# rdpoor/pygmu2

Hardware: AMD Instinct MI355X
Metric: Msamples/s rendered (benchmark_pes.py metric: output frames / wall second) (higher is better)
Workload: dtype f64; 1 GPU; C2: BiquadPE(SinePE(440), lowpass 1 kHz, q 0.707), 44.1 kHz mono, render(start, 1_000_000) per step; frames_counted=11287000000, parallelism=single chain, c2_process_warmup_streams=10

## Files before the change

include/pygmu_hip.h:

```cpp
#ifndef PYGMU_HIP_H
#define PYGMU_HIP_H

#include <stddef.h>
#include <stdint.h>

#define PGX_HOST

#ifdef __cplusplus
extern "C" {
#endif

typedef enum {
    PGX_OK = 0,
    PGX_ERR_INVALID = -1,
    PGX_ERR_RUNTIME = -2,
    PGX_ERR_NOT_INIT = -3,
    PGX_ERR_NOMEM = -4
} pgx_status;

int pgx_abi_version(void);
const char *pgx_last_error(void);
int pgx_device_count(PGX_HOST int *count);
int pgx_init(int device);
int pgx_shutdown(void);
// ... 60 lines not shown
    int32_t pad;
} pgx_sine_stateful_params;
int pgx_sine_stateful(float *out, int64_t n, int channels, double sample_rate,
                      const pgx_sine_stateful_params *params,
                      const float *freq, const float *amp, const float *phase_mod,
                      double *state );

size_t pgx_sine_stateful_bank_workspace_bytes(int64_t n, int batch);
int pgx_sine_stateful_bank(float *out, int64_t out_stride, int batch, int64_t n, int channels, double sample_rate,
                           const pgx_sine_stateful_params *params ,
                           const float *freq, int64_t freq_stride, const float *amp, int64_t amp_stride,
                           const float *phase_mod, int64_t phase_stride,
                           double *state , void *workspace );

int pgx_gain_const(float *out, const float *in, int64_t n_elems, float gain);
int pgx_gain_vec(float *out, const float *in, const float *gain, int64_t n, int channels,
                 int gain_channels );
int pgx_mix_n(float *out, PGX_HOST const float *const *ins_host, int k, int64_t n_elems);
int pgx_mix_batch(float *out, const float *in, int64_t in_stride, int batch, int64_t n_elems);
int pgx_gain_mix_batch(float *out, const float *in, int64_t in_stride, const float *gain,
                       int64_t gain_stride, int batch, int64_t n, int channels, int gain_channels);

size_t pgx_biquad_workspace_bytes(int batch, int64_t n, int channels, int64_t settle_frames);
size_t pgx_biquad_table_doubles(void);
int pgx_biquad_tables(double *tables, const double *coef , int batch);
int pgx_biquad_const(float *out, int64_t out_stride, const float *in, int64_t in_stride,
                     int batch, int64_t n, int channels,
                     const double *coef , const double *tables, int64_t settle_frames,
                     double *state , void *workspace);

int pgx_biquad_sine_supported(int64_t n, int64_t settle_frames);
int pgx_biquad_sine(float *out, int64_t start, int64_t n, double sample_rate, double w, double amp, double phase0,
                    const double *coef , const double *tables, int64_t settle_frames,
                    double *state ,
                    double *state_backup );
int pgx_biquad_sine_set_runs(int min_chunks);
int pgx_biquad_sine_runs_plan(int64_t n, int64_t settle_frames, PGX_HOST int out[5]);
int pgx_biquad_sine_set_pacing(int mode);
int pgx_biquad_sine_pacing_info(int64_t out[3]);

int pgx_biquad_tone_supported(int64_t n, int64_t settle_frames, double w, double sample_rate, double b0, double b1,
                              double b2, double a1, double a2);
double pgx_biquad_tone_gain(double w, double sample_rate, double b0, double b1, double b2, double a1, double a2);
double pgx_biquad_tone_l1(int64_t settle_frames, double b0, double b1, double b2, double a1, double a2);
int pgx_biquad_tone(float *out, int64_t start, int64_t n, double sample_rate, double w, double amp, double phase0,
                    double b0, double b1, double b2, double a1, double a2, const double *tables,
                    int64_t settle_frames, double *state , double *state_backup );
int64_t pgx_biquad_tone_window_frames(void);
void *pgx_biquad_tone_plan(double sample_rate, double w, double amp, double phase0, double b0, double b1, double b2,
                           double a1, double a2, const double *tables, int64_t settle_frames);
int pgx_biquad_tone_plan_free(void *plan);
int pgx_biquad_tone_window(const void *plan, float *out, int64_t start, int64_t n, double *state ,
                           double *state_backup );

typedef struct {
    double freq;
    double q;
    double gain_db;
    int32_t mode;
    int32_t pad;
} pgx_biquad_var_params;
size_t pgx_scan2_workspace_bytes(int64_t n, int channels);
int pgx_biquad_varying(float *out, const float *in, int64_t n, int channels, double sample_rate,
                       const pgx_biquad_var_params *params, const float *freq, const float *q,
                       double gain_a, double gain_sqrt_a, double *state ,
                       void *workspace);
int pgx_biquad_varying_bank(float *out, int64_t out_stride, const float *in, int64_t in_stride, int batch, int64_t n,
                            int channels, double sample_rate, const pgx_biquad_var_params *params, const double *gains,
                            const float *freq, int64_t freq_stride, const float *q, int64_t q_stride,
                            double *state, void *workspace);

int pgx_svf(float *out, const float *in, int64_t n, int channels, double sample_rate,
            const pgx_biquad_var_params *params, const float *freq, const float *q, double gain_a,
            const double *coef ,
            double *state , void *workspace );
int pgx_svf_bank(float *out, int64_t out_stride, const float *in, int64_t in_stride, int batch, int64_t n, int channels,
                 double sample_rate, const pgx_biquad_var_params *params, const double *gains,
                 const float *freq, int64_t freq_stride, const float *q, int64_t q_stride, const double *coef,
                 double *state, void *workspace);

size_t pgx_envelope_scratch_bytes(int64_t n, int channels);
int pgx_envelope(float *out, const float *in, int64_t n, int channels, double attack_coeff,
                 double release_coeff, int one_pole, int rms_window, int64_t rms_period, double *state,
                 double *scratch);

typedef struct {
    int32_t code;
    int32_t pad;
    double p0;
    double p1;
} pgx_transform_op;
int pgx_transform(float *out, const float *in, int64_t n_elems, const pgx_transform_op *ops, int nops);
int pgx_transform_bank(float *out, const float *in, int64_t per_voice, int batch, const pgx_transform_op *ops,
                       int nops);

typedef struct {
    int32_t code;
    int32_t tuning;
    double p0;
    double p1;
} pgx_tuning_op;
typedef struct {
    double reference_pitch;
    double reference_freq;
    double divisions;
    int64_t table_offset;
// ... 375 lines not shown
```

pygmu2_amd/biquad_pe.py:

```python

from __future__ import annotations

from enum import Enum

import ctypes
import math
import os

import numpy as np

from . import device as _dev
from . import diagnostics as _diag
from ._kernels import DeviceBuffer, check, lib, new_output, ptr
from .config import handle_error
from .extent import Extent
from .processing_element import ProcessingElement
from .sine_pe import SinePE
from .snippet import Snippet

FUSE_SINE_SOURCE = True
SINE_FAST_RANGE = 2.0e9
TONE_WINDOWS = os.environ.get("PYGMU_BIQUAD_TONE", "1") != "0"


def tone_window_frames() -> int:
    return int(_dev.load_library().pgx_biquad_tone_window_frames())


class _TonePlan:
    __slots__ = ("handle",)

    def __init__(self, handle):
        self.handle = handle

    def __del__(self):
        handle, self.handle = self.handle, None
        if handle:
            try:
                _dev.load_library().pgx_biquad_tone_plan_free(handle)
            except Exception:
                pass


class BiquadMode(Enum):
    LOWPASS = "lowpass"
    HIGHPASS = "highpass"
    BANDPASS = "bandpass"
    NOTCH = "notch"
    ALLPASS = "allpass"
    PEAKING = "peaking"
    LOWSHELF = "lowshelf"
    HIGHSHELF = "highshelf"


_MODE_INDEX = {m: i for i, m in enumerate(BiquadMode)}


def rbj_coefficients(mode: BiquadMode, freq: float, q: float, gain_db: float, sample_rate: float):
    f = np.atleast_1d(freq).astype(np.float64)
    qq = np.atleast_1d(q).astype(np.float64)
    nyquist = sample_rate / 2.0
    f = np.clip(f, 1.0, nyquist * 0.99)
    qq = np.clip(qq, 0.01, 100.0)
    omega = 2.0 * np.pi * f / sample_rate
    sn, cs = np.sin(omega), np.cos(omega)
    alpha = sn / (2.0 * qq)
    A = 10.0 ** (gain_db / 40.0)
    if mode == BiquadMode.LOWPASS:
        b0 = (1.0 - cs) / 2.0; b1 = 1.0 - cs; b2 = (1.0 - cs) / 2.0
        a0 = 1.0 + alpha; a1 = -2.0 * cs; a2 = 1.0 - alpha
    elif mode == BiquadMode.HIGHPASS:
        b0 = (1.0 + cs) / 2.0; b1 = -(1.0 + cs); b2 = (1.0 + cs) / 2.0
        a0 = 1.0 + alpha; a1 = -2.0 * cs; a2 = 1.0 - alpha
    elif mode == BiquadMode.BANDPASS:
        b0 = alpha; b1 = 0.0; b2 = -alpha
        a0 = 1.0 + alpha; a1 = -2.0 * cs; a2 = 1.0 - alpha
    elif mode == BiquadMode.NOTCH:
        b0 = 1.0; b1 = -2.0 * cs; b2 = 1.0
        a0 = 1.0 + alpha; a1 = -2.0 * cs; a2 = 1.0 - alpha
# ... 135 lines not shown
            self._state.zero_()

    _on_start = _reset_state
    _on_stop = _reset_state

    def _ensure_state(self, channels: int) -> None:
        if self._state is None or self._state_channels != channels:
            per = 4 if (self._freq_is_pe or self._q_is_pe) else 2
            self._state = DeviceBuffer((channels, per), np.float64, zero=True)
            self._state_channels = channels

    def _prepare_constant(self, L, sr: float) -> None:
        if self._coef is None:
            coef = rbj_coefficients(self._mode, self._frequency, self._q, self._gain_db, sr)
            self._coef = DeviceBuffer.from_host(np.asarray(coef, dtype=np.float64))
            self._coef_host = tuple(float(c) for c in coef)
            self._settle = settle_frames(coef[3], coef[4])
            if self._settle:
                self._tables = DeviceBuffer((L.pgx_biquad_table_doubles(),), np.float64)
                check(L.pgx_biquad_tables(self._tables.ptr, self._coef.ptr, 1), "pgx_biquad_tables")

    def _sine_chain(self):
        if self._sine_chain_memo is None:
            src, chain = self._source, False
            if (not self._freq_is_pe and not self._q_is_pe and type(src) is SinePE and not src._has_pe_inputs()
                    and src._channels == 1):
                L = lib()
                sr = float(self.sample_rate)
                self._prepare_constant(L, sr)
                w = 2.0 * np.pi * float(src._frequency)
                if self._settle and _passes_more_signal_than_rounding(self._coef_host, w / sr, self._settle):
                    chain = (w, float(src._amplitude), float(src._phase))
            self._sine_chain_memo = chain
        return self._sine_chain_memo or None

    def _render_sine_source(self, start: int, duration: int):
        if not FUSE_SINE_SOURCE or _diag.is_enabled():
            return None
        chain = self._sine_chain()
        if chain is None:
            return None
        w, amp, phase = chain
        L = lib()
        sr = float(self.sample_rate)
        ok = self._sine_supported.get(duration)
        if ok is None:
            ok = self._sine_supported[duration] = bool(L.pgx_biquad_sine_supported(duration, self._settle))
        if not ok or abs(phase) + abs(w) * ((abs(start) + duration) / sr) >= SINE_FAST_RANGE:
            return None
        self._ensure_state(1)
        out = new_output(duration, 1)
        backup, self._backup_target = self._backup_target, None
        if self._takes_tone_window(L, start, duration, w, phase, sr):
            plan = self._tone_plan
            if plan is None:
                plan = self._tone_plan = _TonePlan(L.pgx_biquad_tone_plan(sr, w, amp, phase, *self._coef_host,
                                                                          self._tables.ptr, self._settle))
            check(L.pgx_biquad_tone_window(plan.handle, out.ptr, start, duration, self._state.ptr, ptr(backup)),
                  "pgx_biquad_tone_window")
            return Snippet(start, out)
        check(L.pgx_biquad_sine(out.ptr, start, duration, sr, w, amp, phase, self._coef.ptr, self._tables.ptr,
                                self._settle, self._state.ptr, ptr(backup)), "pgx_biquad_sine")
        return Snippet(start, out)

    def _takes_tone_window(self, L, start: int, duration: int, w: float, phase: float, sr: float) -> bool:
        if not TONE_WINDOWS:
            return False
        ok = self._tone_supported.get(duration)
        if ok is None:
            plan = (ctypes.c_int * 5)()
            ok = self._tone_supported[duration] = bool(
                L.pgx_biquad_sine_runs_plan(duration, self._settle, plan)
                and L.pgx_biquad_tone_supported(duration, self._settle, w, sr, *self._coef_host))
        return ok and abs(phase) + abs(w) * ((abs(start) + duration + 1) / sr) + 8.0 < SINE_FAST_RANGE

    def _look_ahead_frames(self):
        if not (TONE_WINDOWS and FUSE_SINE_SOURCE) or _diag.is_enabled():
            return None
        if self._tone_hint is None:
            frames, chain = tone_window_frames(), self._sine_chain()
            ok = False
            if frames > 0 and chain is not None:
                L = lib()
                plan = (ctypes.c_int * 5)()
                ok = bool(L.pgx_biquad_sine_runs_plan(frames, self._settle, plan)
                          and L.pgx_biquad_tone_supported(frames, self._settle, chain[0], float(self.sample_rate),
                                                          *self._coef_host))
            self._tone_hint = (frames if ok else None,)
        return self._tone_hint[0]

    def _la_take_snapshot(self):
        if self._state is None or self._sine_chain() is None or not FUSE_SINE_SOURCE:
            return None
        ring = self._backup_ring
        if len(ring) < 3 or ring[0].shape != self._state.shape:
            ring[:] = [DeviceBuffer(self._state.shape, self._state.dtype) for _ in range(3)]
        for _ in range(3):
            self._backup_turn = (self._backup_turn + 1) % 3
            target = ring[self._backup_turn]
            if target is not self._state:
                break
        self._backup_target = target
        return {"_state": target, "_state_channels": self._state_channels}

    def _flush_backup(self) -> None:
        backup, self._backup_target = self._backup_target, None
        if backup is not None and self._state is not None:
            check(lib().pgx_memcpy_d2d(backup.ptr, self._state.ptr, backup.nbytes), "pgx_memcpy_d2d")

    def _render(self, start: int, duration: int) -> Snippet:
        fused = self._render_sine_source(start, duration)
        if fused is not None:
            return fused
        if self._backup_target is not None:
            self._flush_backup()
        src = self._source.render(start, duration)
# ... 43 lines not shown
```

pygmu2_amd/csrc/_fast.c:

```c
#define PY_SSIZE_T_CLEAN
#include <Python.h>
#include <structmember.h>

static PyObject *g_snippet_type, *g_window_type, *g_slow_render, *g_slow_del, *g_diag_dict;
static PyObject *s_la_win, *s_ra_win, *s_la_last, *s_ra_last, *s_active, *s_shape;
static Py_ssize_t sn_start, sn_host, sn_dev, sn_shape, sn_ready, sn_copy, sn_base, sn_bank;
static Py_ssize_t w_first, w_end, w_buf, w_served, w_block;

#define SLOT(obj, off) (*(PyObject **)((char *)(obj) + (off)))

static Py_ssize_t slot_offset(PyObject *type, const char *name) {
    PyObject *d = PyObject_GetAttrString(type, name);
    if (!d) return -1;
    if (Py_TYPE(d) != &PyMemberDescr_Type) {
        Py_DECREF(d);
        PyErr_Format(PyExc_TypeError, "%s is not a __slots__ member", name);
        return -1;
    }
    const Py_ssize_t off = ((PyMemberDescrObject *)d)->d_member->offset;
    Py_DECREF(d);
    return off;
}

static void set_slot(PyObject *o, Py_ssize_t off, PyObject *v) {
    Py_INCREF(v);
    SLOT(o, off) = v;
}

static PyObject *make_row(PyObject *start, PyObject *window, long long first_row, PyObject *rows) {
    PyObject *shape_w = PyObject_GetAttr(window, s_shape);
    if (!shape_w) return NULL;
    if (!PyTuple_Check(shape_w) || PyTuple_GET_SIZE(shape_w) < 2) {
        Py_DECREF(shape_w);
        PyErr_SetString(PyExc_ValueError, "window must be a (frames, channels) buffer");
        return NULL;
    }
    PyObject *shape = PyTuple_Pack(2, rows, PyTuple_GET_ITEM(shape_w, 1));
    Py_DECREF(shape_w);
    if (!shape) return NULL;
    PyObject *row0 = PyLong_FromLongLong(first_row);
    PyObject *base = row0 ? PyTuple_Pack(2, window, row0) : NULL;
    Py_XDECREF(row0);
    if (!base) {
        Py_DECREF(shape);
        return NULL;
    }
    PyTypeObject *tp = (PyTypeObject *)g_snippet_type;
    PyObject *o = tp->tp_alloc(tp, 0);
    if (!o) {
        Py_DECREF(shape);
        Py_DECREF(base);
        return NULL;
    }
    set_slot(o, sn_start, start);
    set_slot(o, sn_ready, Py_None);
    set_slot(o, sn_copy, Py_None);
    set_slot(o, sn_host, Py_None);
    set_slot(o, sn_dev, Py_None);
    SLOT(o, sn_base) = base;
    SLOT(o, sn_shape) = shape;
    set_slot(o, sn_bank, Py_False);
    return o;
}

static PyObject *call_slow(PyObject *self, PyObject *const *args, Py_ssize_t nargs, PyObject *kwnames) {
    const Py_ssize_t nkw = kwnames ? PyTuple_GET_SIZE(kwnames) : 0;
    PyObject *stack[8];
    if (nargs + nkw + 1 > 8) {
        PyErr_SetString(PyExc_TypeError, "render() takes (start, duration)");
        return NULL;
    }
    stack[0] = self;
    for (Py_ssize_t i = 0; i < nargs + nkw; ++i) stack[1 + i] = args[i];
    return PyObject_Vectorcall(g_slow_render, stack, (size_t)(nargs + 1), kwnames);
}

static int as_ll(PyObject *v, long long *out) {
    int overflow = 0;
    *out = PyLong_AsLongLongAndOverflow(v, &overflow);
    return !overflow && !(*out == -1 && PyErr_Occurred());
}

static PyObject *fast_render(PyObject *self, PyObject *const *args, Py_ssize_t nargs, PyObject *kwnames) {
    if (nargs == 2 && !kwnames && PyLong_CheckExact(args[0]) && PyLong_CheckExact(args[1])) {
        long long s, d;
        PyObject *active = PyDict_GetItem(g_diag_dict, s_active);
        if (as_ll(args[0], &s) && as_ll(args[1], &d) && d > 0 && active && PyLong_CheckExact(active) &&
            Py_SIZE(active) == 0) {
            PyObject **dictptr = _PyObject_GetDictPtr(self);
            PyObject *dict = dictptr ? *dictptr : NULL;
            if (dict) {
                PyObject *win = PyDict_GetItem(dict, s_la_win);
                if (win) {
                    if ((PyObject *)Py_TYPE(win) == g_window_type) {
                        long long served, end, first, blk;
                        PyObject *buf = SLOT(win, w_buf);
                        if (buf && SLOT(win, w_served) && SLOT(win, w_end) && SLOT(win, w_first) && SLOT(win, w_block) &&
                            as_ll(SLOT(win, w_served), &served) && as_ll(SLOT(win, w_end), &end) &&
                            as_ll(SLOT(win, w_first), &first) && as_ll(SLOT(win, w_block), &blk) && s == served &&
                            s + d <= end && (blk == 0 || d == blk)) {
                            PyObject *now = PyLong_FromLongLong(s + d);
                            if (!now) return NULL;
                            PyObject *old = SLOT(win, w_served);
                            Py_INCREF(now);
                            SLOT(win, w_served) = now;
                            Py_DECREF(old);
                            const int rc = PyDict_SetItem(dict, s_la_last, now);
                            Py_DECREF(now);
                            if (rc < 0) return NULL;
                            return make_row(args[0], buf, s - first, args[1]);
                        }
                    }
                    PyErr_Clear();
                } else {
                    win = PyDict_GetItem(dict, s_ra_win);
                    if (win && PyTuple_CheckExact(win) && (PyTuple_GET_SIZE(win) == 3 || PyTuple_GET_SIZE(win) == 4)) {
                        long long first, end, period = 0;
                        const int on_grid = PyTuple_GET_SIZE(win) == 3 ||
                                            (as_ll(PyTuple_GET_ITEM(win, 3), &period) && period > 0 && d == period);
                        if (on_grid && as_ll(PyTuple_GET_ITEM(win, 0), &first) && as_ll(PyTuple_GET_ITEM(win, 1), &end) &&
                            first <= s && s + d <= end && (period == 0 || (s - first) % period == 0)) {
                            PyObject *now = PyLong_FromLongLong(s + d);
                            if (!now) return NULL;
                            const int rc = PyDict_SetItem(dict, s_ra_last, now);
                            Py_DECREF(now);
                            if (rc < 0) return NULL;
                            return make_row(args[0], PyTuple_GET_ITEM(win, 2), s - first, args[1]);
                        }
                        PyErr_Clear();
                    }
                }
            }
        }
        if (PyErr_Occurred()) PyErr_Clear();
    }
    return call_slow(self, args, nargs, kwnames);
}

static PyObject *fast_del(PyObject *self, PyObject *ignored) {
    PyObject *ready = SLOT(self, sn_ready), *copy = SLOT(self, sn_copy);
    if ((ready == NULL || ready == Py_None) && (copy == NULL || copy == Py_None)) Py_RETURN_NONE;
    return PyObject_CallOneArg(g_slow_del, self);
}

static PyObject *py_window_rows(PyObject *module, PyObject *const *args, Py_ssize_t nargs) {
    long long first;
    if (nargs != 4 || !as_ll(args[2], &first)) {
        if (!PyErr_Occurred()) PyErr_SetString(PyExc_TypeError, "window_rows(start, window, first_row, rows)");
        return NULL;
    }
    return make_row(args[0], args[1], first, args[3]);
}

static PyMethodDef render_def = {"render", (PyCFunction)(void (*)(void))fast_render, METH_FASTCALL | METH_KEYWORDS,
                                 "render(start, duration) -> Snippet (hot exits in C, else the Python implementation)"};
static PyMethodDef del_def = {"__del__", (PyCFunction)fast_del, METH_NOARGS, "Snippet finalizer (fast exit in C)"};

static PyObject *py_install(PyObject *module, PyObject *args) {
    PyObject *pe_type, *snippet_type, *window_type, *slow_render, *slow_del, *diag_dict;
    if (!PyArg_ParseTuple(args, "OOOOOO", &pe_type, &snippet_type, &window_type, &slow_render, &slow_del, &diag_dict))
        return NULL;
    if (!PyType_Check(pe_type) || !PyType_Check(snippet_type) || !PyType_Check(window_type) || !PyDict_Check(diag_dict)) {
        PyErr_SetString(PyExc_TypeError, "install(PE type, Snippet type, _Window type, slow render, slow del, dict)");
        return NULL;
    }
#define OFF(var, type, name) if ((var = slot_offset(type, name)) < 0) return NULL
    OFF(sn_start, snippet_type, "_start"); OFF(sn_host, snippet_type, "_host"); OFF(sn_dev, snippet_type, "_dev");
    OFF(sn_shape, snippet_type, "_shape"); OFF(sn_ready, snippet_type, "_ready"); OFF(sn_copy, snippet_type, "_copy");
    OFF(sn_base, snippet_type, "_base"); OFF(sn_bank, snippet_type, "_bank_window");
    OFF(w_first, window_type, "first"); OFF(w_end, window_type, "end"); OFF(w_buf, window_type, "buf");
    OFF(w_served, window_type, "served"); OFF(w_block, window_type, "block");
#undef OFF
    Py_INCREF(snippet_type); Py_INCREF(window_type); Py_INCREF(slow_render); Py_INCREF(slow_del); Py_INCREF(diag_dict);
    g_snippet_type = snippet_type; g_window_type = window_type; g_slow_render = slow_render; g_slow_del = slow_del;
    g_diag_dict = diag_dict;
    PyObject *d = PyDescr_NewMethod((PyTypeObject *)pe_type, &render_def);
    if (!d || PyObject_SetAttrString(pe_type, "render", d) < 0) {
        Py_XDECREF(d);
        return NULL;
    }
    Py_DECREF(d);
    d = PyDescr_NewMethod((PyTypeObject *)snippet_type, &del_def);
    if (!d || PyObject_SetAttrString(snippet_type, "__del__", d) < 0) {
        Py_XDECREF(d);
        return NULL;
    }
    Py_DECREF(d);
    Py_RETURN_TRUE;
}

static PyMethodDef module_methods[] = {
    {"install", py_install, METH_VARARGS, "install the C render() / __del__ on the given classes"},
    {"window_rows", (PyCFunction)(void (*)(void))py_window_rows, METH_FASTCALL,
     "window_rows(start, window, first_row, rows) -> Snippet (as Snippet.window_rows)"},
    {NULL, NULL, 0, NULL}};

static struct PyModuleDef moduledef = {PyModuleDef_HEAD_INIT, "_fast", "hot host paths of pygmu2_amd in C", -1,
                                       module_methods};

PyMODINIT_FUNC PyInit__fast(void) {
    s_la_win = PyUnicode_InternFromString("_la_win");
    s_ra_win = PyUnicode_InternFromString("_ra_win");
    s_la_last = PyUnicode_InternFromString("_la_last");
    s_ra_last = PyUnicode_InternFromString("_ra_last");
    s_active = PyUnicode_InternFromString("_ACTIVE");
    s_shape = PyUnicode_InternFromString("shape");
    if (!s_la_win || !s_ra_win || !s_la_last || !s_ra_last || !s_active || !s_shape) return NULL;
    return PyModule_Create(&moduledef);
}
```

pygmu2_amd/csrc/pgx_tone.hip:

```cpp
#include "pgx_common.h"

#include <cmath>

#ifndef PGX_TONE_GROUPS
#define PGX_TONE_GROUPS 4
#endif
#ifndef PGX_TONE_STORE_AUX
#define PGX_TONE_STORE_AUX 16
#endif

namespace {

constexpr int kToneBlock = 256;
constexpr int kToneGroups = PGX_TONE_GROUPS;
constexpr int kToneGroupStride = kToneBlock * 4;
constexpr int kTonePiece = kToneGroupStride * kToneGroups;
constexpr int kTabWave = 24, kTabLane = 28, kTabRows = 28 + 4 * 64, kTabDoubles = kTabRows + 2 * 16;
constexpr double kToneNoiseRatio = 4.0;

struct ToneArgs {
    double w, amp, phase0, sr, inv_sr;
    double phase_t;
    double gain;
    double hr, hi;
    double cos_d, sin_d;
    double two_cos_d;
    double cos_g, sin_g;
    double b1, b2, a1, a2;
    int64_t start, settle;
};

typedef unsigned int tone_v4u __attribute__((ext_vector_type(4)));

__device__ __forceinline__ void tone_steady_state(const ToneArgs &a, int64_t m, double &zx, double &zy) {
    double x0 = 0.0, y0 = 0.0, x1 = 0.0, y1 = 0.0;
#pragma nounroll
    for (int k = 0; k < 2; ++k) {
        const double t = pgx::pgx_div_by((double)(m - 1 + k), a.sr, a.inv_sr);
        double sn, cs;
        pgx::pgx_sincos_bounded(a.phase0 + a.w * t, sn, cs);
        x0 = x1;
        y0 = y1;
        x1 = (double)(float)(a.amp * sn);
        y1 = __builtin_fma(a.hr, sn, a.hi * cs);
    }
    zy = a.b2 * x1 - a.a2 * y1;
    zx = (a.b2 * x0 - a.a2 * y0) + (a.b1 * x1 - a.a1 * y1);
}

template <bool HEAD>
__device__ __forceinline__ void tone_piece(float *__restrict__ out, int64_t n, const double *__restrict__ tables,
                                           const ToneArgs &a, int64_t piece, bool aligned, double dzx, double dzy) {
    const int tid = threadIdx.x;
    const int64_t p0 = piece * kTonePiece;
    const int64_t f0 = p0 + 4 * tid;
    if (f0 >= n) return;
    double sn, cs;
    {
        const double t = pgx::pgx_div_by((double)(a.start + f0), a.sr, a.inv_sr);
        pgx::pgx_sincos_bounded(a.phase_t + a.w * t, sn, cs);
    }
    sn *= a.gain;
    cs *= a.gain;
    const int64_t left = n - p0;
    const uint64_t base = (uint64_t)(out + p0);
    const uint32_t lo = __builtin_amdgcn_readfirstlane((uint32_t)base), hi = __builtin_amdgcn_readfirstlane((uint32_t)(base >> 32));
    __amdgpu_buffer_rsrc_t rsrc = __builtin_amdgcn_make_buffer_rsrc(
        (void *)(((uint64_t)hi << 32) | lo), 0, (int)(left < kTonePiece ? left : kTonePiece) * 4, 0x00020000);
#pragma unroll
    for (int u = 0; u < kToneGroups; ++u) {
        const int64_t f = f0 + (int64_t)u * kToneGroupStride;
        double y[4];
        y[0] = sn;
        y[1] = __builtin_fma(cs, a.sin_d, sn * a.cos_d);
        if (PGX_HOT(a.two_cos_d != 0.0)) {
            y[2] = __builtin_fma(a.two_cos_d, y[1], -y[0]);
            y[3] = __builtin_fma(a.two_cos_d, y[2], -y[1]);
        } else {
            const double c1 = __builtin_fma(-sn, a.sin_d, cs * a.cos_d);
            y[2] = __builtin_fma(c1, a.sin_d, y[1] * a.cos_d);
            const double c2 = __builtin_fma(-y[1], a.sin_d, c1 * a.cos_d);
            y[3] = __builtin_fma(c2, a.sin_d, y[2] * a.cos_d);
        }
        if (HEAD && PGX_COLD(f < a.settle)) {
            const int k = (int)(f >> 10), q = (int)(f >> 4) & 63, r = (int)f & 15;
            double vx = dzx, vy = dzy;
            const double *pw = tables + kTabWave;
            for (int kk = 0; kk < k; ++kk) {
                const double nx = __builtin_fma(pw[0], vx, pw[1] * vy);
                vy = __builtin_fma(pw[2], vx, pw[3] * vy);
                vx = nx;
            }
            const double *pq = tables + kTabLane + 4 * q;
            const double qx = __builtin_fma(pq[0], vx, pq[1] * vy), qy = __builtin_fma(pq[2], vx, pq[3] * vy);
            const double *rows = tables + kTabRows + 2 * r;
#pragma unroll
            for (int j = 0; j < 4; ++j) y[j] += __builtin_fma(rows[2 * j], qx, rows[2 * j + 1] * qy);
        }
        if (f < n) {
            if (PGX_HOT(aligned && f + 4 <= n)) {
                const tone_v4u v = {__float_as_uint((float)y[0]), __float_as_uint((float)y[1]),
                                    __float_as_uint((float)y[2]), __float_as_uint((float)y[3])};
                __builtin_amdgcn_raw_buffer_store_b128(v, rsrc, (tid * 4 + u * kToneGroupStride) * 4, 0,
                                                       PGX_TONE_STORE_AUX );
            } else {
#pragma unroll
                for (int j = 0; j < 4; ++j)
                    if (f + j < n) out[f + j] = (float)y[j];
            }
        }
        if (u + 1 < kToneGroups) {
            const double s2 = __builtin_fma(cs, a.sin_g, sn * a.cos_g);
            cs = __builtin_fma(-sn, a.sin_g, cs * a.cos_g);
            sn = s2;
        }
    }
}

__global__ void __launch_bounds__(kToneBlock, 8)
k_biquad_tone(float *__restrict__ out, int64_t n, const double *__restrict__ tables, double *state,
              double *state_backup, ToneArgs a) {
    const bool aligned = ((uintptr_t)out & 15) == 0;
    if (blockIdx.x != 0) {
        tone_piece<false>(out, n, tables, a, (int64_t)blockIdx.x, aligned, 0.0, 0.0);
        return;
    }
    const double sx = state[0], sy = state[1];
    double zx = 0.0, zy = 0.0, ex = 0.0, ey = 0.0;
#pragma nounroll
    for (int k = 0; k < 2; ++k) {
        zx = ex;
        zy = ey;
        tone_steady_state(a, k == 0 ? a.start - 1 : a.start + n - 1, ex, ey);
    }
    __syncthreads();
    if (threadIdx.x == 0) {
        if (state_backup) {
            state_backup[0] = sx;
            state_backup[1] = sy;
        }
        state[0] = ex;
        state[1] = ey;
    }
    tone_piece<true>(out, n, tables, a, 0, aligned, sx - zx, sy - zy);
}

struct ToneFilter {
    double w, sr, b0, b1, b2, a1, a2;
    long double hr, hi;
    double gain;
    int64_t l1_frames;
    double l1;
};

static long double tone_response(double w, double sr, double b0, double b1, double b2, double a1, double a2,
                                 long double &hr, long double &hi) {
    const long double d = (long double)w / (long double)sr;
    const long double c1 = cosl(d), s1 = -sinl(d), c2 = cosl(2.0L * d), s2 = -sinl(2.0L * d);
    const long double nr = b0 + b1 * c1 + b2 * c2, ni = b1 * s1 + b2 * s2;
    const long double dr = 1.0L + a1 * c1 + a2 * c2, di = a1 * s1 + a2 * s2;
    const long double den = dr * dr + di * di;
    hr = (nr * dr + ni * di) / den;
    hi = (ni * dr - nr * di) / den;
    return hypotl(hr, hi);
}

static double tone_l1(int64_t frames, double b0, double b1, double b2, double a1, double a2) {
    double s0 = 0.0, s1 = 0.0, l1 = 0.0, x = 1.0;
    for (int64_t i = 0; i < frames; ++i) {
        const double y = s0 + b0 * x;
        s0 = s1 + b1 * x - a1 * y;
        s1 = b2 * x - a2 * y;
        l1 += fabs(y);
        x = 0.0;
    }
    return l1;
}

static ToneFilter &tone_filter(double w, double sr, double b0, double b1, double b2, double a1, double a2) {
    static ToneFilter f{};
    static bool have = false;
    if (!have || f.w != w || f.sr != sr || f.b0 != b0 || f.b1 != b1 || f.b2 != b2 || f.a1 != a1 || f.a2 != a2) {
        f = ToneFilter{w, sr, b0, b1, b2, a1, a2, 0.0L, 0.0L, 0.0, 0, 0.0};
        f.gain = (double)tone_response(w, sr, b0, b1, b2, a1, a2, f.hr, f.hi);
        have = true;
    }
    return f;
}

static bool tone_supported(int64_t n, int64_t settle, double w, double sr, double b0, double b1, double b2, double a1,
                           double a2) {
    if (settle <= 0 || settle > kTonePiece || n < 2 * settle || !(sr > 0.0)) return false;
    if (!(fabs(w) * ((double)n / sr) < pgx::kSinFastRange)) return false;
    ToneFilter &f = tone_filter(w, sr, b0, b1, b2, a1, a2);
    if (f.l1_frames != settle) {
        f.l1 = tone_l1(settle, b0, b1, b2, a1, a2);
        f.l1_frames = settle;
    }
    return std::isfinite(f.gain) && std::isfinite(f.l1) && f.l1 <= kToneNoiseRatio * f.gain;
}

constexpr int64_t kToneWindowFrames = 36000000;

static int64_t tone_window_frames_env() {
    const char *e = getenv("PGX_TONE_WINDOW_FRAMES");
    if (e && *e) {
        char *end = nullptr;
        const long long v = strtoll(e, &end, 10);
        if (end != e && v >= 0) return (int64_t)v;
    }
    return kToneWindowFrames;
}

struct TonePlan {
    ToneArgs a;
    const double *tables;
    double phase_abs, w_abs;
};

static bool tone_make_plan(TonePlan &p, double sample_rate, double w, double amp, double phase0, double b0, double b1,
                           double b2, double a1, double a2, const double *tables, int64_t settle_frames) {
    if (!tables || !(sample_rate > 0.0)) return false;
    if (!tone_supported(2 * settle_frames, settle_frames, w, sample_rate, b0, b1, b2, a1, a2)) return false;
    const ToneFilter &f = tone_filter(w, sample_rate, b0, b1, b2, a1, a2);
    static ToneArgs cached;
    static bool have = false;
    if (!have || cached.w != w || cached.sr != sample_rate) {
        ToneArgs c{};
        c.w = w;
        c.sr = sample_rate;
        c.inv_sr = 1.0 / sample_rate;
        const long double d = (long double)w / (long double)sample_rate;
        c.cos_d = (double)cosl(d);
        c.sin_d = (double)sinl(d);
        c.two_cos_d = (fabsl(sinl(d)) >= 1e-3L) ? (double)(2.0L * cosl(d)) : 0.0;
        const long double turn = 6.283185307179586476925286766559L;
        long double g = d * (long double)kToneGroupStride;
        g -= turn * floorl(g / turn);
        c.cos_g = (double)cosl(g);
        c.sin_g = (double)sinl(g);
        cached = c;
        have = true;
    }
    ToneArgs a = cached;
    a.amp = amp;
    a.phase0 = phase0;
    a.phase_t = phase0 + (double)atan2l(f.hi, f.hr);
    a.gain = amp * f.gain;
    a.hr = amp * (double)f.hr;
    a.hi = amp * (double)f.hi;
    a.b1 = b1;
    a.b2 = b2;
    a.a1 = a1;
    a.a2 = a2;
    a.start = 0;
    a.settle = settle_frames;
    p.a = a;
    p.tables = tables;
    p.phase_abs = fabs(phase0);
    p.w_abs = fabs(w);
    return true;
}

static int tone_launch(const TonePlan &p, float *out, int64_t start, int64_t n, double *state, double *state_backup,
                       const char *who) {
    PGX_CHECK_ARG(out && state, std::string(who) + ": bad argument");
    PGX_CHECK_ARG(pgx_biquad_table_doubles() == (size_t)kTabDoubles, std::string(who) + ": table layout changed");
    PGX_CHECK_ARG(n >= 2 * p.a.settle && p.w_abs * ((double)n / p.a.sr) < pgx::kSinFastRange,
                  std::string(who) + ": chain or block not supported (pgx_biquad_tone_supported)");
    const double far = p.phase_abs + p.w_abs * ((double)(llabs(start) + n + 1) / p.a.sr);
    PGX_CHECK_ARG(far + 4.0 < pgx::kSinFastRange, std::string(who) + ": phase beyond the fast sine range");
    ToneArgs a = p.a;
    a.start = start;
    const int64_t pieces = pgx::ceil_div(n, (int64_t)kTonePiece);
    PGX_CHECK_ARG(pieces <= 0x7fffffff, std::string(who) + ": block too long");
    hipLaunchKernelGGL(k_biquad_tone, dim3((unsigned)pieces), dim3(kToneBlock), 0, pgx::stream(), out, n, p.tables, state,
                       state_backup, a);
    PGX_LAUNCH_CHECK("k_biquad_tone");
    return PGX_OK;
}

}

extern "C" {

int pgx_biquad_tone_supported(int64_t n, int64_t settle_frames, double w, double sample_rate, double b0, double b1,
                              double b2, double a1, double a2) {
    return tone_supported(n, settle_frames, w, sample_rate, b0, b1, b2, a1, a2) ? 1 : 0;
}

double pgx_biquad_tone_gain(double w, double sample_rate, double b0, double b1, double b2, double a1, double a2) {
    long double hr, hi;
    return (double)tone_response(w, sample_rate, b0, b1, b2, a1, a2, hr, hi);
}

double pgx_biquad_tone_l1(int64_t settle_frames, double b0, double b1, double b2, double a1, double a2) {
    return tone_l1(settle_frames, b0, b1, b2, a1, a2);
}

int64_t pgx_biquad_tone_window_frames(void) {
    static const int64_t frames = tone_window_frames_env();
    return frames;
}

void *pgx_biquad_tone_plan(double sample_rate, double w, double amp, double phase0, double b0, double b1, double b2,
                           double a1, double a2, const double *tables, int64_t settle_frames) {
    TonePlan *p = new TonePlan;
    if (!tone_make_plan(*p, sample_rate, w, amp, phase0, b0, b1, b2, a1, a2, tables, settle_frames)) {
        delete p;
        return nullptr;
    }
    return p;
}

int pgx_biquad_tone_plan_free(void *plan) {
    delete static_cast<TonePlan *>(plan);
    return PGX_OK;
}

int pgx_biquad_tone_window(const void *plan, float *out, int64_t start, int64_t n, double *state, double *state_backup) {
    PGX_REQUIRE_INIT();
    if (n <= 0) return PGX_OK;
    PGX_CHECK_ARG(plan, "pgx_biquad_tone_window: no plan");
    return tone_launch(*static_cast<const TonePlan *>(plan), out, start, n, state, state_backup, "pgx_biquad_tone_window");
}

int pgx_biquad_tone(float *out, int64_t start, int64_t n, double sample_rate, double w, double amp, double phase0,
                    double b0, double b1, double b2, double a1, double a2, const double *tables,
                    int64_t settle_frames, double *state, double *state_backup) {
    PGX_REQUIRE_INIT();
    if (n <= 0) return PGX_OK;
    PGX_CHECK_ARG(out && tables && state && sample_rate > 0, "pgx_biquad_tone: bad argument");
    TonePlan p;
    PGX_CHECK_ARG(tone_make_plan(p, sample_rate, w, amp, phase0, b0, b1, b2, a1, a2, tables, settle_frames),
                  "pgx_biquad_tone: chain or block not supported (pgx_biquad_tone_supported)");
    return tone_launch(p, out, start, n, state, state_backup, "pgx_biquad_tone");
}

}
```

pygmu2_amd/look_ahead.py:

```python

from __future__ import annotations

import os
import threading

import numpy as np

from . import read_ahead as _read_ahead

SMALL_BLOCK = 1 << 20
FIRST_WINDOW_BLOCKS = 8
WINDOW_GROWTH = 2
AHEAD_BLOCKS = int(os.environ.get("PGX_LOOK_AHEAD_BLOCKS", "256"))
AHEAD_FRAMES = int(os.environ.get("PGX_LOOK_AHEAD_FRAMES", str(1 << 25)))
AHEAD_FRAMES_SMALL_GRAPH = int(os.environ.get("PGX_LOOK_AHEAD_FRAMES_SMALL", str(1 << 27)))
_FRAMES_EXPLICIT = "PGX_LOOK_AHEAD_FRAMES" in os.environ


def frame_cap(n_nodes: int) -> int:
    if _FRAMES_EXPLICIT or n_nodes > 4:
        return AHEAD_FRAMES
    return max(AHEAD_FRAMES, AHEAD_FRAMES_SMALL_GRAPH if n_nodes <= 2 else AHEAD_FRAMES_SMALL_GRAPH // 2)


# ... 92 lines not shown
        return type(value)(value)
    return value


def _snapshot_plan(nodes):
    plan = []
    for pe in nodes:
        fields = getattr(pe, "_STATE_FIELDS", None)
        if fields:
            plan.append((pe, fields, getattr(pe, "_la_take_snapshot", None)))
    return plan


def take_snapshot(nodes, plan=None):
    snap = []
    for pe, fields, own in (plan if plan is not None else _snapshot_plan(nodes)):
        saved = own() if own is not None else None
        if saved is None:
            saved = {name: _copy_value(getattr(pe, name)) for name in fields}
        snap.append((pe, saved))
    return snap


def restore_snapshot(snap) -> None:
    for pe, fields in snap:
        for name, value in fields.items():
            setattr(pe, name, value)


def _flush_pending_backups(snap) -> None:
    for n, _ in snap:
        if getattr(n, "_backup_target", None) is not None:
            n._flush_backup()


def _expected_window_failure(exc) -> bool:
    return isinstance(exc, (_read_ahead.Declined, MemoryError, ValueError))


_noted: set = set()


def _note_window_failure(pe, exc) -> None:
    key = (type(pe).__name__, type(exc).__name__, str(exc)[:80])
    if key not in _noted:
        _noted.add(key)
        import logging
        logging.getLogger("pygmu2_amd.look_ahead").warning(
            "%s: look-ahead window declined (%s: %s); this PE renders block by block from here on",
            type(pe).__name__, type(exc).__name__, exc)


class _Window:
    __slots__ = ("first", "end", "buf", "served", "snap", "nodes", "block")


def render(pe, start: int, duration: int):
    if _busy():
        return None
    d = pe.__dict__
    owner = d.get("_la_owner")
    if owner is not None:
        settle(owner)
    win = d.get("_la_win")
    if not _ENABLED:
        if win is not None:
            settle(pe)
        return None
    if win is not None:
        if start == win.served and start + duration <= win.end and (not win.block or duration == win.block):
            win.served = start + duration
            d["_la_last"] = win.served
            from .snippet import Snippet
            return Snippet.window_rows(start, win.buf, start - win.first, duration)
        settle(pe)
    if duration > SMALL_BLOCK or not capable(pe):
        return None
    sequential = d.get("_la_last") == start
    d["_la_last"] = start + duration
    if not sequential:
        d["_la_grow"] = FIRST_WINDOW_BLOCKS
        return None
    from .snippet import Snippet
    nodes = d.get("_la_nodes")
    if nodes is None:
        nodes = []
        _subtree(pe, set(), nodes)
        d["_la_nodes"] = nodes
        d["_la_plan"] = _snapshot_plan(nodes)
        d["_la_below"] = [n for n in nodes if n is not pe]
    for n in d["_la_below"]:
        if "_la_win" in n.__dict__:
            settle(n)
    snap = take_snapshot(nodes, d["_la_plan"])
    block = duration if d.get("_la_sensitive") else 0
    _tls.busy = True
    _tls.period = block
    grow = d.get("_la_grow", FIRST_WINDOW_BLOCKS)
    hint = getattr(pe, "_look_ahead_frames", None)
    blocks = window_blocks(grow, duration, len(nodes), hint() if hint is not None else None)
    try:
        big = pe._render(start, duration * blocks)
    except BaseException as exc:
        _tls.busy = False
        _tls.period = 0
        d["_la_ok"] = False
        try:
            _flush_pending_backups(snap)
            restore_snapshot(snap)
        except Exception:
            if _expected_window_failure(exc):
                raise
        if not _expected_window_failure(exc):
            raise
        _note_window_failure(pe, exc)
        return None
    finally:
        _tls.busy = False
        _tls.period = 0
    _flush_pending_backups(snap)
    d["_la_grow"] = grow * WINDOW_GROWTH
    STATS["window_frames"] += duration * blocks
    STATS["windows"] += 1
    if not big.on_device:
        restore_snapshot(snap)
        _tls.busy = True
        try:
            return pe._render(start, duration)
        finally:
            _tls.busy = False
    win = _Window()
    win.first, win.end, win.buf = start, start + big.duration, big.dev
    win.served, win.snap, win.nodes, win.block = start + duration, snap, nodes, block
    d["_la_win"] = win
    for n in d["_la_below"]:
        n.__dict__["_la_owner"] = pe
    return Snippet.window_rows(start, win.buf, 0, duration)


def settle(owner) -> None:
    win = owner.__dict__.pop("_la_win", None)
    if win is None:
        return
    for n in win.nodes:
        if n.__dict__.get("_la_owner") is owner:
            del n.__dict__["_la_owner"]
    if win.served >= win.end:
        return
    restore_snapshot(win.snap)
    if win.served > win.first:
        was = _busy()
        _tls.busy = True
        _tls.period = win.block
        try:
            owner._render(win.first, win.served - win.first)
        finally:
            _tls.busy = was
            _tls.period = 0


def before_direct_access(pe) -> None:
    if _busy():
        return
    owner = pe.__dict__.get("_la_owner")
    if owner is not None:
        settle(owner)
    if pe.__dict__.get("_la_win") is not None:
        settle(pe)


def forget(pe) -> None:
    pe.__dict__.pop("_la_last", None)
```

pygmu2_amd/processing_element.py:

```python

from __future__ import annotations

import time
from abc import ABC, abstractmethod

import numpy as np

from . import device as _dev
from . import diagnostics as _diag
from . import look_ahead as _look_ahead
from . import read_ahead as _read_ahead
from .config import get_sample_rate, handle_error
from .diagnostics import is_enabled, pull_count_enabled, record_pull, record_timing, timing_enabled
from .extent import Extent
from .snippet import Snippet


_RA_LIMIT = _read_ahead.SMALL_BLOCK
_LA_LIMIT = _look_ahead.SMALL_BLOCK


class ProcessingElement(ABC):
    _sample_rate: int | None = None
    _cached_extent: Extent | None = None
    _READ_AHEAD_SAFE = False

    def __new__(cls, *args, **kwargs):
        rate = get_sample_rate()
        if rate is None:
            raise RuntimeError(
                "Global sample_rate is required but not set. "
                "Call pygmu2_amd.set_sample_rate(rate) before constructing PEs.")
        obj = super().__new__(cls)
        obj._sample_rate = rate
        return obj

    @property
    def sample_rate(self) -> int | None:
        if self._sample_rate is not None:
            return self._sample_rate
        found = None
        for pe in self.inputs():
            r = pe.sample_rate
            if r is None:
                continue
            if found is None:
                found = r
            elif found != r:
                handle_error(f"{type(self).__name__}.sample_rate inferred conflicting input rates: "
                             f"{found} vs {r}. Using {found}.", fatal=False)
                break
        return found

    def render(self, start: int, duration: int) -> Snippet:
        if duration <= 0:
            if duration < 0:
                raise ValueError(f"duration must be >= 0, got {duration}")
        elif not _diag._ACTIVE:
            d = self.__dict__
            win = d.get("_la_win")
            if win is not None:
                end = start + duration
                if start == win.served and end <= win.end and (not win.block or duration == win.block):
                    win.served = d["_la_last"] = end
                    return Snippet.window_rows(start, win.buf, start - win.first, duration)
            else:
                win = d.get("_ra_win")
                if (win is not None and win[0] <= start and start + duration <= win[1]
                        and (len(win) == 3 or (duration == win[3] and (start - win[0]) % win[3] == 0))):
                    d["_ra_last"] = start + duration
                    return Snippet.window_rows(start, win[2], start - win[0], duration)
        diag = is_enabled() if _diag._ACTIVE else False
        if diag and pull_count_enabled():
            record_pull(self)
        if duration == 0:
            ch = self.channel_count()
            return Snippet.from_zeros(start, 0, int(ch) if ch is not None else 1)
        if diag and timing_enabled():
            if "_la_win" in self.__dict__ or "_la_owner" in self.__dict__:
                _look_ahead.before_direct_access(self)
            t0 = time.perf_counter_ns()
            out = self._render(start, duration)
            record_timing(self, time.perf_counter_ns() - t0)
            return out
        if duration <= _RA_LIMIT:
            d = self.__dict__
            win = d.get("_ra_win")
            if (win is not None and win[0] <= start and start + duration <= win[1]
                    and (len(win) == 3 or (duration == win[3] and (start - win[0]) % win[3] == 0))):
                d["_ra_last"] = start + duration
                return Snippet.window_rows(start, win[2], start - win[0], duration)
            if d.get("_ra_ok", True):
                ahead = _read_ahead.render(self, start, duration)
                if ahead is not None:
                    return ahead
            if (duration <= _LA_LIMIT and d.get("_la_ok", True)) or "_la_win" in d or "_la_owner" in d:
                ahead = _look_ahead.render(self, start, duration)
                if ahead is not None:
                    return ahead
        elif "_la_win" in self.__dict__ or "_la_owner" in self.__dict__:
            _look_ahead.before_direct_access(self)
        return self._render(start, duration)

    @abstractmethod
    def _render(self, start: int, duration: int) -> Snippet:
        ...

    @abstractmethod
    def inputs(self) -> list["ProcessingElement"]:
        ...

    def extent(self) -> Extent:
        if self._cached_extent is None:
            self._cached_extent = self._compute_extent()
        return self._cached_extent

    def _compute_extent(self) -> Extent:
        return Extent(None, None)
# ... 93 lines not shown
```

Measured before the change: 1.642 million Msamples/s.

## Split look-ahead tone window output into main buffer plus separate tail block

Adds a split variant of the fused sine+biquad tone kernel that writes the last block of a look-ahead window into a separate buffer. The look-ahead window and the C fast path serve rows from either the main buffer or the tail, so the final block can live in its own allocation, presumably to avoid keeping or copying one huge window buffer when the next window starts. The default window size is also raised from 36M to 64M frames to amortise launch and Python overhead over more frames. In exchange, the kernel gains extra branches for pieces that straddle the split, and larger windows use more device memory.

```diff
diff --git a/include/pygmu_hip.h b/include/pygmu_hip.h
--- a/include/pygmu_hip.h
+++ b/include/pygmu_hip.h
@@ -136,6 +136,9 @@
 int pgx_biquad_tone_plan_free(void *plan);
 int pgx_biquad_tone_window(const void *plan, float *out, int64_t start, int64_t n, double *state ,
                            double *state_backup );
+int pgx_biquad_tone_window_split(const void *plan, float *out, float *out_tail, int64_t tail_frames, int64_t start,
+                                 int64_t n, double *state , double *state_backup );
+int pgx_biquad_tone_split_tail(void);
 
 typedef struct {
     double freq;
diff --git a/pygmu2_amd/biquad_pe.py b/pygmu2_amd/biquad_pe.py
--- a/pygmu2_amd/biquad_pe.py
+++ b/pygmu2_amd/biquad_pe.py
@@ -25,6 +25,16 @@
 
 def tone_window_frames() -> int:
     return int(_dev.load_library().pgx_biquad_tone_window_frames())
+
+
+_SPLIT_TAIL = None
+
+
+def tone_split_tail() -> bool:
+    global _SPLIT_TAIL
+    if _SPLIT_TAIL is None:
+        _SPLIT_TAIL = bool(_dev.load_library().pgx_biquad_tone_split_tail())
+    return _SPLIT_TAIL
 
 
 class _TonePlan:
@@ -266,16 +276,45 @@
         out = new_output(duration, 1)
         backup, self._backup_target = self._backup_target, None
         if self._takes_tone_window(L, start, duration, w, phase, sr):
-            plan = self._tone_plan
-            if plan is None:
-                plan = self._tone_plan = _TonePlan(L.pgx_biquad_tone_plan(sr, w, amp, phase, *self._coef_host,
-                                                                          self._tables.ptr, self._settle))
+            plan = self._tone_window_plan(L, sr, w, amp, phase)
             check(L.pgx_biquad_tone_window(plan.handle, out.ptr, start, duration, self._state.ptr, ptr(backup)),
                   "pgx_biquad_tone_window")
             return Snippet(start, out)
         check(L.pgx_biquad_sine(out.ptr, start, duration, sr, w, amp, phase, self._coef.ptr, self._tables.ptr,
                                 self._settle, self._state.ptr, ptr(backup)), "pgx_biquad_sine")
         return Snippet(start, out)
+
+    def _tone_window_plan(self, L, sr: float, w: float, amp: float, phase: float) -> _TonePlan:
+        plan = self._tone_plan
+        if plan is None:
+            plan = self._tone_plan = _TonePlan(L.pgx_biquad_tone_plan(sr, w, amp, phase, *self._coef_host,
+                                                                      self._tables.ptr, self._settle))
+        return plan
+
+    def _render_window(self, start: int, duration: int, blocks: int):
+        if blocks < 2 or not FUSE_SINE_SOURCE or _diag.is_enabled():
+            return None
+        chain = self._sine_chain()
+        if chain is None or not tone_split_tail():
+            return None
+        w, amp, phase = chain
+        L = lib()
+        sr = float(self.sample_rate)
+        n = duration * blocks
+        ok = self._sine_supported.get(n)
+        if ok is None:
+            ok = self._sine_supported[n] = bool(L.pgx_biquad_sine_supported(n, self._settle))
+        if not ok or abs(phase) + abs(w) * ((abs(start) + n) / sr) >= SINE_FAST_RANGE:
+            return None
+        if not self._takes_tone_window(L, start, n, w, phase, sr):
+            return None
+        self._ensure_state(1)
+        out, tail = new_output(n - duration, 1), new_output(duration, 1)
+        backup, self._backup_target = self._backup_target, None
+        plan = self._tone_window_plan(L, sr, w, amp, phase)
+        check(L.pgx_biquad_tone_window_split(plan.handle, out.ptr, tail.ptr, duration, start, n, self._state.ptr,
+                                             ptr(backup)), "pgx_biquad_tone_window_split")
+        return Snippet(start, out), tail
 
     def _takes_tone_window(self, L, start: int, duration: int, w: float, phase: float, sr: float) -> bool:
         if not TONE_WINDOWS:
diff --git a/pygmu2_amd/csrc/_fast.c b/pygmu2_amd/csrc/_fast.c
--- a/pygmu2_amd/csrc/_fast.c
+++ b/pygmu2_amd/csrc/_fast.c
@@ -5,7 +5,7 @@
 static PyObject *g_snippet_type, *g_window_type, *g_slow_render, *g_slow_del, *g_diag_dict;
 static PyObject *s_la_win, *s_ra_win, *s_la_last, *s_ra_last, *s_active, *s_shape;
 static Py_ssize_t sn_start, sn_host, sn_dev, sn_shape, sn_ready, sn_copy, sn_base, sn_bank;
-static Py_ssize_t w_first, w_end, w_buf, w_served, w_block;
+static Py_ssize_t w_first, w_end, w_split, w_tail, w_buf, w_served, w_block;
 
 #define SLOT(obj, off) (*(PyObject **)((char *)(obj) + (off)))
 
@@ -93,12 +93,15 @@
                 PyObject *win = PyDict_GetItem(dict, s_la_win);
                 if (win) {
                     if ((PyObject *)Py_TYPE(win) == g_window_type) {
-                        long long served, end, first, blk;
-                        PyObject *buf = SLOT(win, w_buf);
+                        long long served, end, first, blk, split = 0;
+                        PyObject *buf = SLOT(win, w_buf), *tail = SLOT(win, w_tail);
+                        const int has_tail = tail && tail != Py_None;
                         if (buf && SLOT(win, w_served) && SLOT(win, w_end) && SLOT(win, w_first) && SLOT(win, w_block) &&
                             as_ll(SLOT(win, w_served), &served) && as_ll(SLOT(win, w_end), &end) &&
                             as_ll(SLOT(win, w_first), &first) && as_ll(SLOT(win, w_block), &blk) && s == served &&
-                            s + d <= end && (blk == 0 || d == blk)) {
+                            s + d <= end && (blk == 0 || d == blk) &&
+                            (!has_tail || (SLOT(win, w_split) && as_ll(SLOT(win, w_split), &split) &&
+                                           (s + d <= split || s >= split)))) {
                             PyObject *now = PyLong_FromLongLong(s + d);
                             if (!now) return NULL;
                             PyObject *old = SLOT(win, w_served);
@@ -108,6 +111,7 @@
                             const int rc = PyDict_SetItem(dict, s_la_last, now);
                             Py_DECREF(now);
                             if (rc < 0) return NULL;
+                            if (has_tail && s >= split) return make_row(args[0], tail, s - split, args[1]);
                             return make_row(args[0], buf, s - first, args[1]);
                         }
                     }
@@ -168,7 +172,8 @@
     OFF(sn_start, snippet_type, "_start"); OFF(sn_host, snippet_type, "_host"); OFF(sn_dev, snippet_type, "_dev");
     OFF(sn_shape, snippet_type, "_shape"); OFF(sn_ready, snippet_type, "_ready"); OFF(sn_copy, snippet_type, "_copy");
     OFF(sn_base, snippet_type, "_base"); OFF(sn_bank, snippet_type, "_bank_window");
-    OFF(w_first, window_type, "first"); OFF(w_end, window_type, "end"); OFF(w_buf, window_type, "buf");
+    OFF(w_first, window_type, "first"); OFF(w_end, window_type, "end"); OFF(w_split, window_type, "split");
+    OFF(w_tail, window_type, "tail"); OFF(w_buf, window_type, "buf");
     OFF(w_served, window_type, "served"); OFF(w_block, window_type, "block");
 #undef OFF
     Py_INCREF(snippet_type); Py_INCREF(window_type); Py_INCREF(slow_render); Py_INCREF(slow_del); Py_INCREF(diag_dict);
diff --git a/pygmu2_amd/csrc/pgx_tone.hip b/pygmu2_amd/csrc/pgx_tone.hip
--- a/pygmu2_amd/csrc/pgx_tone.hip
+++ b/pygmu2_amd/csrc/pgx_tone.hip
@@ -48,13 +48,26 @@
     zx = (a.b2 * x0 - a.a2 * y0) + (a.b1 * x1 - a.a1 * y1);
 }
 
-template <bool HEAD>
+template <bool HEAD, bool SPLIT>
 __device__ __forceinline__ void tone_piece(float *__restrict__ out, int64_t n, const double *__restrict__ tables,
-                                           const ToneArgs &a, int64_t piece, bool aligned, double dzx, double dzy) {
+                                           const ToneArgs &a, int64_t piece, bool aligned, double dzx, double dzy,
+                                           float *__restrict__ tail, int64_t split, bool tail_aligned) {
     const int tid = threadIdx.x;
     const int64_t p0 = piece * kTonePiece;
     const int64_t f0 = p0 + 4 * tid;
     if (f0 >= n) return;
+    float *dst = out + p0;
+    int64_t lim = n;
+    bool straddle = false;
+    if (SPLIT) {
+        if (p0 >= split) {
+            dst = tail + (p0 - split);
+            aligned = tail_aligned;
+        } else {
+            lim = split;
+            straddle = split < p0 + kTonePiece;
+        }
+    }
     double sn, cs;
     {
         const double t = pgx::pgx_div_by((double)(a.start + f0), a.sr, a.inv_sr);
@@ -62,11 +75,20 @@
     }
     sn *= a.gain;
     cs *= a.gain;
-    const int64_t left = n - p0;
-    const uint64_t base = (uint64_t)(out + p0);
+    const int64_t left = lim - p0;
+    const uint64_t base = (uint64_t)dst;
     const uint32_t lo = __builtin_amdgcn_readfirstlane((uint32_t)base), hi = __builtin_amdgcn_readfirstlane((uint32_t)(base >> 32));
     __amdgpu_buffer_rsrc_t rsrc = __builtin_amdgcn_make_buffer_rsrc(
         (void *)(((uint64_t)hi << 32) | lo), 0, (int)(left < kTonePiece ? left : kTonePiece) * 4, 0x00020000);
+    __amdgpu_buffer_rsrc_t rsrc_tail = rsrc;
+    if (SPLIT && straddle) {
+        const uint64_t tbase = (uint64_t)tail;
+        const uint32_t tlo = __builtin_amdgcn_readfirstlane((uint32_t)tbase),
+                       thi = __builtin_amdgcn_readfirstlane((uint32_t)(tbase >> 32));
+        const int64_t end = n - p0 < kTonePiece ? n : p0 + kTonePiece;
+        rsrc_tail = __builtin_amdgcn_make_buffer_rsrc((void *)(((uint64_t)thi << 32) | tlo), 0, (int)(end - split) * 4,
+                                                      0x00020000);
+    }
 #pragma unroll
     for (int u = 0; u < kToneGroups; ++u) {
         const int64_t f = f0 + (int64_t)u * kToneGroupStride;
@@ -98,15 +120,37 @@
             for (int j = 0; j < 4; ++j) y[j] += __builtin_fma(rows[2 * j], qx, rows[2 * j + 1] * qy);
         }
         if (f < n) {
-            if (PGX_HOT(aligned && f + 4 <= n)) {
+            if (SPLIT && PGX_COLD(straddle)) {
+                const tone_v4u v = {__float_as_uint((float)y[0]), __float_as_uint((float)y[1]),
+                                    __float_as_uint((float)y[2]), __float_as_uint((float)y[3])};
+                if (aligned && f + 4 <= split) {
+                    __builtin_amdgcn_raw_buffer_store_b128(v, rsrc, (tid * 4 + u * kToneGroupStride) * 4, 0,
+                                                           PGX_TONE_STORE_AUX );
+                } else if (tail_aligned && f >= split && f + 4 <= n) {
+                    __builtin_amdgcn_raw_buffer_store_b128(v, rsrc_tail, (int)(f - split) * 4, 0,
+                                                           PGX_TONE_STORE_AUX );
+                } else {
+#pragma unroll
+                    for (int j = 0; j < 4; ++j) {
+                        const int64_t g = f + j;
+                        if (g < split) out[g] = (float)y[j];
+                        else if (g < n) tail[g - split] = (float)y[j];
+                    }
+                }
+            } else if (PGX_HOT(aligned && f + 4 <= lim)) {
                 const tone_v4u v = {__float_as_uint((float)y[0]), __float_as_uint((float)y[1]),
                                     __float_as_uint((float)y[2]), __float_as_uint((float)y[3])};
                 __builtin_amdgcn_raw_buffer_store_b128(v, rsrc, (tid * 4 + u * kToneGroupStride) * 4, 0,
                                                        PGX_TONE_STORE_AUX );
             } else {
 #pragma unroll
-                for (int j = 0; j < 4; ++j)
-                    if (f + j < n) out[f + j] = (float)y[j];
+                for (int j = 0; j < 4; ++j) {
+                    if (SPLIT) {
+                        if (f + j < lim) dst[f - p0 + j] = (float)y[j];
+                    } else {
+                        if (f + j < n) out[f + j] = (float)y[j];
+                    }
+                }
             }
         }
         if (u + 1 < kToneGroups) {
@@ -117,12 +161,14 @@
     }
 }
 
-__global__ void __launch_bounds__(kToneBlock, 8)
-k_biquad_tone(float *__restrict__ out, int64_t n, const double *__restrict__ tables, double *state,
-              double *state_backup, ToneArgs a) {
+template <bool SPLIT>
+__device__ __forceinline__ void tone_block(float *__restrict__ out, int64_t n, const double *__restrict__ tables,
+                                           double *state, double *state_backup, const ToneArgs &a,
+                                           float *__restrict__ tail, int64_t split) {
     const bool aligned = ((uintptr_t)out & 15) == 0;
+    const bool tail_aligned = SPLIT && ((uintptr_t)tail & 15) == 0 && (split & 3) == 0;
     if (blockIdx.x != 0) {
-        tone_piece<false>(out, n, tables, a, (int64_t)blockIdx.x, aligned, 0.0, 0.0);
+        tone_piece<false, SPLIT>(out, n, tables, a, (int64_t)blockIdx.x, aligned, 0.0, 0.0, tail, split, tail_aligned);
         return;
     }
     const double sx = state[0], sy = state[1];
@@ -142,7 +188,19 @@
         state[0] = ex;
         state[1] = ey;
     }
-    tone_piece<true>(out, n, tables, a, 0, aligned, sx - zx, sy - zy);
+    tone_piece<true, SPLIT>(out, n, tables, a, 0, aligned, sx - zx, sy - zy, tail, split, tail_aligned);
+}
+
+__global__ void __launch_bounds__(kToneBlock, 8)
+k_biquad_tone(float *__restrict__ out, int64_t n, const double *__restrict__ tables, double *state,
+              double *state_backup, ToneArgs a) {
+    tone_block<false>(out, n, tables, state, state_backup, a, nullptr, n);
+}
+
+__global__ void __launch_bounds__(kToneBlock, 8)
+k_biquad_tone_split(float *__restrict__ out, float *__restrict__ tail, int64_t split, int64_t n,
+                    const double *__restrict__ tables, double *state, double *state_backup, ToneArgs a) {
+    tone_block<true>(out, n, tables, state, state_backup, a, tail, split);
 }
 
 struct ToneFilter {
@@ -200,7 +258,7 @@
     return std::isfinite(f.gain) && std::isfinite(f.l1) && f.l1 <= kToneNoiseRatio * f.gain;
 }
 
-constexpr int64_t kToneWindowFrames = 36000000;
+constexpr int64_t kToneWindowFrames = 64000000;
 
 static int64_t tone_window_frames_env() {
     const char *e = getenv("PGX_TONE_WINDOW_FRAMES");
@@ -263,8 +321,10 @@
 }
 
 static int tone_launch(const TonePlan &p, float *out, int64_t start, int64_t n, double *state, double *state_backup,
-                       const char *who) {
-    PGX_CHECK_ARG(out && state, std::string(who) + ": bad argument");
+                       const char *who, float *out_tail = nullptr, int64_t tail_frames = 0) {
+    PGX_CHECK_ARG(tail_frames >= 0 && tail_frames <= n, std::string(who) + ": tail_frames outside [0, n]");
+    PGX_CHECK_ARG(tail_frames == 0 || out_tail, std::string(who) + ": tail frames and no out_tail");
+    PGX_CHECK_ARG((out || tail_frames == n) && state, std::string(who) + ": bad argument");
     PGX_CHECK_ARG(pgx_biquad_table_doubles() == (size_t)kTabDoubles, std::string(who) + ": table layout changed");
     PGX_CHECK_ARG(n >= 2 * p.a.settle && p.w_abs * ((double)n / p.a.sr) < pgx::kSinFastRange,
                   std::string(who) + ": chain or block not supported (pgx_biquad_tone_supported)");
@@ -274,6 +334,12 @@
     a.start = start;
     const int64_t pieces = pgx::ceil_div(n, (int64_t)kTonePiece);
     PGX_CHECK_ARG(pieces <= 0x7fffffff, std::string(who) + ": block too long");
+    if (tail_frames > 0) {
+        hipLaunchKernelGGL(k_biquad_tone_split, dim3((unsigned)pieces), dim3(kToneBlock), 0, pgx::stream(), out, out_tail,
+                           n - tail_frames, n, p.tables, state, state_backup, a);
+        PGX_LAUNCH_CHECK("k_biquad_tone_split");
+        return PGX_OK;
+    }
     hipLaunchKernelGGL(k_biquad_tone, dim3((unsigned)pieces), dim3(kToneBlock), 0, pgx::stream(), out, n, p.tables, state,
                        state_backup, a);
     PGX_LAUNCH_CHECK("k_biquad_tone");
@@ -323,6 +389,25 @@
     if (n <= 0) return PGX_OK;
     PGX_CHECK_ARG(plan, "pgx_biquad_tone_window: no plan");
     return tone_launch(*static_cast<const TonePlan *>(plan), out, start, n, state, state_backup, "pgx_biquad_tone_window");
+}
+
+int pgx_biquad_tone_window_split(const void *plan, float *out, float *out_tail, int64_t tail_frames, int64_t start,
+                                 int64_t n, double *state, double *state_backup) {
+    PGX_REQUIRE_INIT();
+    PGX_CHECK_ARG(tail_frames >= 0 && (n <= 0 || tail_frames <= n), "pgx_biquad_tone_window_split: tail_frames outside [0, n]");
+    PGX_CHECK_ARG(tail_frames == 0 || out_tail, "pgx_biquad_tone_window_split: tail frames and no out_tail");
+    if (n <= 0) return PGX_OK;
+    PGX_CHECK_ARG(plan, "pgx_biquad_tone_window_split: no plan");
+    return tone_launch(*static_cast<const TonePlan *>(plan), out, start, n, state, state_backup,
+                       "pgx_biquad_tone_window_split", out_tail, tail_frames);
+}
+
+int pgx_biquad_tone_split_tail(void) {
+    static const int wanted = []() {
+        const char *e = getenv("PGX_TONE_SPLIT_TAIL");
+        return (e && e[0] == '0' && e[1] == 0) ? 0 : 1;
+    }();
+    return wanted;
 }
 
 int pgx_biquad_tone(float *out, int64_t start, int64_t n, double sample_rate, double w, double amp, double phase0,
diff --git a/pygmu2_amd/look_ahead.py b/pygmu2_amd/look_ahead.py
--- a/pygmu2_amd/look_ahead.py
+++ b/pygmu2_amd/look_ahead.py
@@ -168,7 +168,7 @@
 
 
 class _Window:
-    __slots__ = ("first", "end", "buf", "served", "snap", "nodes", "block")
+    __slots__ = ("first", "end", "buf", "served", "snap", "nodes", "block", "tail", "split")
 
 
 def render(pe, start: int, duration: int):
@@ -185,11 +185,15 @@
         return None
     if win is not None:
         if start == win.served and start + duration <= win.end and (not win.block or duration == win.block):
-            win.served = start + duration
-            d["_la_last"] = win.served
-            from .snippet import Snippet
-            return Snippet.window_rows(start, win.buf, start - win.first, duration)
+            rows = ((win.buf, start - win.first) if getattr(win, "tail", None) is None or start + duration <= win.split
+                    else (win.tail, start - win.split) if start >= win.split else None)
+            if rows is not None:
+                win.served = start + duration
+                d["_la_last"] = win.served
+                from .snippet import Snippet
+                return Snippet.window_rows(start, rows[0], rows[1], duration)
         settle(pe)
+        win = rows = None
     if duration > SMALL_BLOCK or not capable(pe):
         return None
     sequential = d.get("_la_last") == start
@@ -215,8 +219,14 @@
     grow = d.get("_la_grow", FIRST_WINDOW_BLOCKS)
     hint = getattr(pe, "_look_ahead_frames", None)
     blocks = window_blocks(grow, duration, len(nodes), hint() if hint is not None else None)
+    tail = None
     try:
-        big = pe._render(start, duration * blocks)
+        own = getattr(pe, "_render_window", None)
+        parts = own(start, duration, blocks) if own is not None else None
+        if parts is None:
+            big = pe._render(start, duration * blocks)
+        else:
+            big, tail = parts
     except BaseException as exc:
         _tls.busy = False
         _tls.period = 0
@@ -246,7 +256,8 @@
         finally:
             _tls.busy = False
     win = _Window()
-    win.first, win.end, win.buf = start, start + big.duration, big.dev
+    win.first, win.split, win.buf, win.tail = start, start + big.duration, big.dev, tail
+    win.end = win.split + (tail.shape[0] if tail is not None else 0)
     win.served, win.snap, win.nodes, win.block = start + duration, snap, nodes, block
     d["_la_win"] = win
     for n in d["_la_below"]:
diff --git a/pygmu2_amd/processing_element.py b/pygmu2_amd/processing_element.py
--- a/pygmu2_amd/processing_element.py
+++ b/pygmu2_amd/processing_element.py
@@ -62,8 +62,13 @@
             if win is not None:
                 end = start + duration
                 if start == win.served and end <= win.end and (not win.block or duration == win.block):
-                    win.served = d["_la_last"] = end
-                    return Snippet.window_rows(start, win.buf, start - win.first, duration)
+                    tail = getattr(win, "tail", None)
+                    if tail is None or end <= win.split:
+                        win.served = d["_la_last"] = end
+                        return Snippet.window_rows(start, win.buf, start - win.first, duration)
+                    if start >= win.split:
+                        win.served = d["_la_last"] = end
+                        return Snippet.window_rows(start, tail, start - win.split, duration)
             else:
                 win = d.get("_ra_win")
                 if (win is not None and win[0] <= start and start + duration <= win[1]
```

New measurement: 1.766 million Msamples/s, median of 6. 7.6% higher.
